# nubot-nudt/LCR-Net

Hardware: AMD Instinct MI355X
Metric: scans/s (120k-pt KITTI-shape scan -> 256-D descriptor) (higher is better)
Workload: dtype f32 (K-deep GEMMs, K >= 288 and N >= 64: fp32 operands as bf16 x 3 split, 6 of 9 products on the bf16 matrix cores, fp32 accumulate — error vs fp64 <= the fp32-MFMA kernel's; every other GEMM, KPConv and attention: fp32 MFMA); 1 GPU; configs[1]: batch of 8 synthetic 64-beam scans (~120k pts, 0.3 m voxel -> ~16k pts), voxelise + 3 subsamples + 10 radius searches + KPConv encoder + NetVLAD, seeded random weights; distinct_input_batches=4, streams=pre-processing stream (own host thread, 2 batches ahead) + 2 encoder stream(s), parallelism=scan-parallel x1, all-gather of descriptors

## Files before the change

lcr-net_amd/csrc/gemm_f32.hip:

```cpp
#include <cstdio>
#include <cstdlib>
#include <map>
#include <mutex>
#include <type_traits>

#include "common.h"

namespace lcr {

typedef float floatx16 __attribute__((ext_vector_type(16)));

constexpr int GM_BK = 32;
constexpr int GM_T = 256;

constexpr int GM_MAX_BATCH = 64;
struct GemmBatch {
  int     count;
  int     strided;
  int     k[GM_MAX_BATCH];
  int64_t a_off[GM_MAX_BATCH], b_off[GM_MAX_BATCH], c_off[GM_MAX_BATCH];
};

struct GemmEpilogue {
  const float*   bias;
// ... 728 lines not shown
      pin();
      mfma(a1[q], b1[q]);
      pin();
    }
#pragma unroll
    for (int q = 0; q < 4; ++q) {
      if (more && load) {
#pragma unroll
        for (int j = q; j < LPW; j += 4) issue_one(ST, j);
      }
      pin();
      mfma(a2[q], b2[q]);
      pin();
    }
    if (more && load) advance();
    mfma4(fa[3], fb[3]);
    if (more) {
#pragma unroll
      for (int q = 0; q < 4; ++q) fa[q] = na[q], fb[q] = nb[q];
    }
  };
  using I0 = std::integral_constant<int, 0>;
  using I1 = std::integral_constant<int, 1>;
  using I2 = std::integral_constant<int, 2>;
  int t = 0;
  for (; t + 6 <= nk; t += 3) {
    step(I0{}, std::true_type{}, t);
    step(I1{}, std::true_type{}, t + 1);
    step(I2{}, std::true_type{}, t + 2);
  }
  for (; t < nk; t += 3) {
    step(I0{}, std::false_type{}, t);
    if (t + 1 < nk) step(I1{}, std::false_type{}, t + 1);
    if (t + 2 < nk) step(I2{}, std::false_type{}, t + 2);
  }

  floatx16 accs[1] = {acc};
  gemm_epilogue<BM, BN, WM, WN, 1>(accs, C, M, N, m0, n0, m_tile, ep, bias_v, blk_first, blk_seg_start, blk_seg_end, wm, wn, lane);
}

template <int BM, int BN, int WM, int WN>
static int launch_gemm_deep(const float* A, const float* B, float* C, int64_t M, int N, int K, const GemmEpilogue& ep, hipStream_t st,
                            const uint16_t* amask = nullptr, int kshift = 0) {
  const int mt8 = (div_up(M, BM) + 7) / 8 * 8;
  if (amask)
    LCR_LAUNCH_TIMED((k_gemm_f32_deep<BM, BN, WM, WN, true>), dim3(mt8 * div_up(N, BN)), dim3(GM_T), 0, st, A, B, C, M, N, K, ep, amask, kshift);
  else
    LCR_LAUNCH_TIMED((k_gemm_f32_deep<BM, BN, WM, WN>), dim3(mt8 * div_up(N, BN)), dim3(GM_T), 0, st, A, B, C, M, N, K, ep, amask, kshift);
  return check_launch("lcr_gemm_f32");
}

typedef __bf16 bf16x8_t __attribute__((ext_vector_type(8)));
typedef __bf16 bf16x2_t __attribute__((ext_vector_type(2)));
typedef float f32x2_t __attribute__((ext_vector_type(2)));
typedef float f32x4_t __attribute__((ext_vector_type(4)));
typedef uint32_t u32x4_t __attribute__((ext_vector_type(4)));

__device__ __forceinline__ uint32_t pk_bf16(float a, float b) {
  f32x2_t v = {a, b};
  return __builtin_bit_cast(uint32_t, __builtin_convertvector(v, bf16x2_t));
}
__device__ __forceinline__ void split2(float x0, float x1, uint32_t& h1, uint32_t& h2, uint32_t& h3) {
  h1 = pk_bf16(x0, x1);
  const float r0 = fsub(x0, __uint_as_float(h1 << 16)), r1 = fsub(x1, __uint_as_float(h1 & 0xffff0000u));
  h2 = pk_bf16(r0, r1);
  const float s0 = fsub(r0, __uint_as_float(h2 << 16)), s1 = fsub(r1, __uint_as_float(h2 & 0xffff0000u));
  h3 = pk_bf16(s0, s1);
}

__global__ __launch_bounds__(256) void k_split_bf16x3(const float* __restrict__ w, int64_t n, uint16_t* __restrict__ planes) {
  for (int64_t i = (blockIdx.x * static_cast<int64_t>(blockDim.x) + threadIdx.x) * 2; i < n; i += static_cast<int64_t>(gridDim.x) * blockDim.x * 2) {
    const float x0 = w[i], x1 = i + 1 < n ? w[i + 1] : 0.f;
    uint32_t h1, h2, h3;
    split2(x0, x1, h1, h2, h3);
    planes[i] = static_cast<uint16_t>(h1), planes[n + i] = static_cast<uint16_t>(h2), planes[2 * n + i] = static_cast<uint16_t>(h3);
    if (i + 1 < n) planes[i + 1] = static_cast<uint16_t>(h1 >> 16), planes[n + i + 1] = static_cast<uint16_t>(h2 >> 16), planes[2 * n + i + 1] = static_cast<uint16_t>(h3 >> 16);
  }
}

__global__ __launch_bounds__(256) void k_split_bf16x3_tiles(const float* __restrict__ w, int N, int K, uint16_t* __restrict__ tiles) {
  const int KS = K / GM_BK;
  const int64_t blk = blockIdx.x;
  const int ct = static_cast<int>(blk / KS), ks = static_cast<int>(blk % KS);
  const int row = threadIdx.x >> 2, kc = threadIdx.x & 3;
  const int n = ct * 64 + row;
  u32x4_t p1 = {0u, 0u, 0u, 0u}, p2 = p1, p3 = p1;
  if (n < N) {
    const float* src = w + static_cast<int64_t>(n) * K + ks * GM_BK + kc * 8;
    const float4 x0 = ld4(src), x1 = ld4(src + 4);
    uint32_t h1, h2, h3;
    split2(x0.x, x0.y, h1, h2, h3), p1.x = h1, p2.x = h2, p3.x = h3;
    split2(x0.z, x0.w, h1, h2, h3), p1.y = h1, p2.y = h2, p3.y = h3;
    split2(x1.x, x1.y, h1, h2, h3), p1.z = h1, p2.z = h2, p3.z = h3;
    split2(x1.z, x1.w, h1, h2, h3), p1.w = h1, p2.w = h2, p3.w = h3;
  }
  char* dst = reinterpret_cast<char*>(tiles) + blk * 12288 + row * 64 + ((kc ^ ((row >> 2) & 3)) << 4);
  *reinterpret_cast<u32x4_t*>(dst) = p1;
  *reinterpret_cast<u32x4_t*>(dst + 4096) = p2;
  *reinterpret_cast<u32x4_t*>(dst + 8192) = p3;
}

template <int ABL, int NWM, int D = 2, bool MASK = false>
__global__ __launch_bounds__(128 * NWM, 2) void k_gemm_f32_bsplit_p(const float* __restrict__ A, const uint16_t* __restrict__ Bs, float* __restrict__ C,
                                                             int64_t M, int N, int K, GemmEpilogue ep, const uint16_t* __restrict__ amask,
                                                             int kshift) {
  constexpr int BM = 32 * NWM, BN = 64, RS = 64, T = 128 * NWM, PLA = BM * RS, STGA = 3 * PLA, PL = 64 * RS;
  constexpr int NPB = (768 + T - 1) / T;
  constexpr int STG = 3 * PL + (NPB * T - 768) * 16;
  __shared__ __attribute__((aligned(16))) char sA[2 * STGA];
  __shared__ __attribute__((aligned(16))) char sB[2 * STG];
  const int lane = threadIdx.x & 63, w = __builtin_amdgcn_readfirstlane(threadIdx.x >> 6);
  const int wm = w >> 1, wn = w & 1;
  const int ntn = (N + BN - 1) / BN;
  const int xcd = blockIdx.x & 7, slot = blockIdx.x >> 3;
  const int64_t m_tile = static_cast<int64_t>(slot / ntn) * 8 + xcd;
  const int64_t m0 = m_tile * BM;
  const int n0 = (slot % ntn) * BN;
  if (m0 >= M) return;
  const int srow = threadIdx.x >> 3, spc = threadIdx.x & 7;
  const float* ap[2];
  int soff[2];
  uint32_t aoff[2], rmask[2];
#pragma unroll
  for (int j = 0; j < 2; ++j) {
    const int r = srow + j * (T / 8);
    int64_t ga = m0 + r;
    ga = ga < M ? ga : M - 1;
    ap[j] = A + ga * K + spc * 4;
    if constexpr (MASK) {
      aoff[j] = static_cast<uint32_t>((ga * K + spc * 4) * 4);
      rmask[j] = amask[ga];
    } else {
      aoff[j] = rmask[j] = 0;
    }
    soff[j] = r * RS + (((spc >> 1) ^ ((r >> 2) & 3)) << 4) + (spc & 1) * 8;
  }
  const char* bp = reinterpret_cast<const char*>(Bs) + static_cast<int64_t>(n0 / 64) * (K / GM_BK) * 12288;
  int bsrc[NPB], bdst[NPB];
#pragma unroll
  for (int j = 0; j < NPB; ++j) {
    const int q = threadIdx.x + T * j;
    bsrc[j] = (q < 768 ? q : threadIdx.x) * 16;
    bdst[j] = q * 16;
  }
  const int fsw = ((lane & 31) >> 2) & 3, fc0 = ((lane >> 5) ^ fsw) << 4, fc1 = (((lane >> 5) + 2) ^ fsw) << 4;
  const int fa = (wm * 32 + (lane & 31)) * RS, fb = (wn * 32 + (lane & 31)) * RS;
  floatx16 acc, acc2;
#pragma unroll
  for (int r = 0; r < 16; ++r) acc[r] = 0.f, acc2[r] = 0.f;
  const int nk = K / GM_BK;
  f32x4_t ra[D][2];
  u32x4_t rb[D][NPB];
  __amdgpu_buffer_rsrc_t arsrc;
  if constexpr (MASK) arsrc = __builtin_amdgcn_make_buffer_rsrc(const_cast<float*>(A), 0, static_cast<int>(M * K * 4), 0x00020000);
  auto fetch = [&](auto st_c, int t) {
    constexpr int st = decltype(st_c)::value;
    const int tt = t < nk ? t : nk - 1;
    if constexpr (MASK) {
      const int kb = tt >> kshift;
#pragma unroll
      for (int j = 0; j < 2; ++j) {
        const uint32_t o = ((rmask[j] >> kb) & 1u) ? aoff[j] + static_cast<uint32_t>(tt * GM_BK * 4) : 0x80000000u;
        ra[st][j] = __builtin_bit_cast(f32x4_t, __builtin_amdgcn_raw_buffer_load_b128(arsrc, static_cast<int>(o), 0, 0));
      }
    } else {
      ra[st][0] = *reinterpret_cast<const f32x4_t*>(ap[0] + tt * GM_BK), ra[st][1] = *reinterpret_cast<const f32x4_t*>(ap[1] + tt * GM_BK);
    }
#pragma unroll
    for (int j = 0; j < NPB; ++j) rb[st][j] = *reinterpret_cast<const u32x4_t*>(bp + static_cast<int64_t>(tt) * 12288 + bsrc[j]);
  };
  auto park = [&](auto st_c, int lds_stage) {
    constexpr int st = decltype(st_c)::value;
    char* da = sA + lds_stage * STGA;
    char* db = sB + lds_stage * STG;
#pragma unroll
    for (int j = 0; j < 2; ++j) {
      uint32_t h1, h2, h3, g1, g2, g3;
      if constexpr (ABL & 2) {
        h1 = __float_as_uint(ra[st][j].x), h2 = __float_as_uint(ra[st][j].y), h3 = h1, g1 = __float_as_uint(ra[st][j].z), g2 = __float_as_uint(ra[st][j].w), g3 = g1;
      } else {
        split2(ra[st][j].x, ra[st][j].y, h1, h2, h3);
        split2(ra[st][j].z, ra[st][j].w, g1, g2, g3);
      }
      if constexpr (ABL & 4) {
        asm volatile("" ::"v"(h1), "v"(h2), "v"(h3), "v"(g1), "v"(g2), "v"(g3));
      } else {
        *reinterpret_cast<uint2*>(da + soff[j]) = make_uint2(h1, g1);
        *reinterpret_cast<uint2*>(da + PLA + soff[j]) = make_uint2(h2, g2);
        *reinterpret_cast<uint2*>(da + 2 * PLA + soff[j]) = make_uint2(h3, g3);
      }
    }
#pragma unroll
    for (int j = 0; j < NPB; ++j) {
      const u32x4_t v = rb[st][j];
      if constexpr (ABL & 4) {
        asm volatile("" ::"v"(v));
      } else {
        *reinterpret_cast<u32x4_t*>(db + bdst[j]) = v;
      }
    }
  };
  using I0 = std::integral_constant<int, 0>;
  fetch(I0{}, 0);
  if constexpr (D > 1) fetch(std::integral_constant<int, 1 % D>{}, 1);
  if constexpr (D > 2) fetch(std::integral_constant<int, 2 % D>{}, 2);
  if constexpr (D > 3) fetch(std::integral_constant<int, 3 % D>{}, 3);
  float bias_v[1];
  {
    const int col = n0 + wn * 32 + (lane & 31);
    bias_v[0] = (ep.bias && col < N) ? ep.bias[col] : 0.f;
  }
  int blk_first = 0;
  int64_t blk_seg_start = 0, blk_seg_end = 0;
  if (ep.stats != nullptr) {
    blk_seg_end = ep.seg_len[0];
    while (blk_first + 1 < ep.S && m0 >= blk_seg_end) {
      ++blk_first;
      blk_seg_start = blk_seg_end;
      blk_seg_end += ep.seg_len[blk_first];
    }
  }
  park(I0{}, 0);
  fetch(I0{}, D);
  __syncthreads();
  auto step = [&](auto lds_c, auto reg_c, int t) {
    constexpr int P = decltype(lds_c)::value;
    using NX = std::integral_constant<int, (decltype(reg_c)::value + 1) % D>;
    const char* la = sA + P * STGA + fa;
    const char* lb = sB + P * STG + fb;
    bf16x8_t a0[3], b0[3], a1[3], b1[3];
    auto mm = [&](const bf16x8_t& x, const bf16x8_t& y, floatx16& c) {
      if constexpr (ABL & 1) {
        asm volatile("" ::"v"(x), "v"(y));
      } else {
        c = __builtin_amdgcn_mfma_f32_32x32x16_bf16(x, y, c, 0, 0, 0);
      }
    };
    if constexpr (ABL & 16) {
      u32x4_t z = {static_cast<uint32_t>(t), 0u, 0u, 0u};
      asm volatile("" : "+v"(z));
#pragma unroll
      for (int p = 0; p < 3; ++p) a0[p] = b0[p] = a1[p] = b1[p] = __builtin_bit_cast(bf16x8_t, z);
      (void)la, (void)lb;
    } else {
#pragma unroll
      for (int p = 0; p < 3; ++p) {
        a0[p] = __builtin_bit_cast(bf16x8_t, *reinterpret_cast<const u32x4_t*>(la + p * PLA + fc0));
        b0[p] = __builtin_bit_cast(bf16x8_t, *reinterpret_cast<const u32x4_t*>(lb + p * PL + fc0));
      }
#pragma unroll
      for (int p = 0; p < 3; ++p) {
        a1[p] = __builtin_bit_cast(bf16x8_t, *reinterpret_cast<const u32x4_t*>(la + p * PLA + fc1));
        b1[p] = __builtin_bit_cast(bf16x8_t, *reinterpret_cast<const u32x4_t*>(lb + p * PL + fc1));
      }
    }
    mm(a0[2], b0[0], acc);
    mm(a0[0], b0[2], acc2);
    mm(a0[1], b0[1], acc);
    mm(a0[1], b0[0], acc2);
    mm(a0[0], b0[1], acc);
    mm(a0[0], b0[0], acc2);
    park(NX{}, P ^ 1);
    mm(a1[2], b1[0], acc);
    mm(a1[0], b1[2], acc2);
    mm(a1[1], b1[1], acc);
    mm(a1[1], b1[0], acc2);
    mm(a1[0], b1[1], acc);
    mm(a1[0], b1[0], acc2);
    if constexpr (!(ABL & 8)) fetch(NX{}, t + 1 + D);
    __syncthreads();
  };
  static_assert(D == 2 || D == 4, "register stages");
  using I1 = std::integral_constant<int, 1>;
  using I2 = std::integral_constant<int, 2>;
  using I3 = std::integral_constant<int, 3>;
  int t = 0;
  if constexpr (D == 2) {
    for (; t + 2 <= nk; t += 2) {
      step(I0{}, I0{}, t);
      step(I1{}, I1{}, t + 1);
    }
    if (t < nk) step(I0{}, I0{}, t);
  } else {
    for (; t + 4 <= nk; t += 4) {
      step(I0{}, I0{}, t);
      step(I1{}, I1{}, t + 1);
      step(I0{}, I2{}, t + 2);
      step(I1{}, I3{}, t + 3);
    }
    if (t < nk) step(I0{}, I0{}, t);
    if (t + 1 < nk) step(I1{}, I1{}, t + 1);
    if (t + 2 < nk) step(I0{}, I2{}, t + 2);
  }
#pragma unroll
  for (int r = 0; r < 16; ++r) acc[r] += acc2[r];
  floatx16 accs[1] = {acc};
  gemm_epilogue<BM, BN, NWM, 2, 1>(accs, C, M, N, m0, n0, m_tile, ep, bias_v, blk_first, blk_seg_start, blk_seg_end, wm, wn, lane);
}

struct GemmStreamK {
  float*    partial;
  uint32_t* arrived;
  int       U;
};

template <int BM, int BN, int WM, int WN>
__global__ __launch_bounds__(GM_T, 3) void k_gemm_f32_sk(const float* __restrict__ A, const float* __restrict__ B, float* __restrict__ C,
                                                         int64_t M, int N, int K, GemmEpilogue ep, GemmStreamK sk) {
  static_assert(WM * WN == 4 && BM == 32 * WM, "one 32-row MFMA tile per wavefront along M");
  constexpr int LDA = BM + 1, LDB = BN + 4;
  constexpr int NT = BN / (32 * WN);
  __shared__ __attribute__((aligned(16))) float As[2][GM_BK * LDA];
  __shared__ __attribute__((aligned(16))) float Bs[2][GM_BK * LDB];
  const int lane = threadIdx.x & 63, w = __builtin_amdgcn_readfirstlane(threadIdx.x >> 6);
  const int wm = w / WN, wn = w % WN;
  const int ntn = (N + BN - 1) / BN;
  const int64_t mt = (M + BM - 1) / BM;
  const int xcd = blockIdx.x & 7, u = blockIdx.x >> 3;
  const int64_t mt_x = mt > xcd ? (mt - xcd + 7) / 8 : 0;
  const int nk = (K + GM_BK - 1) / GM_BK;
  const int64_t I = mt_x * ntn * nk;
  auto first_it = [&](int uu) { return static_cast<int64_t>(uu) * I / sk.U; };
  const int64_t it_begin = first_it(u), it_end = first_it(u + 1);
  LoaderT<BM, LDA, true> la[2];
  LoaderN<BN, LDB, true> lb[2];
  const int a_off = (lane >> 5) * LDA + wm * 32 + (lane & 31);
  const int b_off = (lane >> 5) * LDB + wn * (32 * NT) + (lane & 31);
  constexpr int PIECE = NT * 16 * GM_T;
  __shared__ unsigned s_arrived;

  int64_t it = it_begin;
  while (it < it_end) {
    const int64_t lt = it / nk;
    const int ks = static_cast<int>(it - lt * nk);
    const int ns = static_cast<int>(min(static_cast<int64_t>(nk - ks), it_end - it));
    const int64_t m_tile = (lt / ntn) * 8 + xcd;
    const int64_t m0 = m_tile * BM;
    const int n0 = static_cast<int>(lt % ntn) * BN;
    const int k_begin = ks * GM_BK;
    auto gload = [&](int k0, int r) {
      la[r].load(A, M, K, m0, k0);
      lb[r].load(B, N, K, n0, k0);
    };
    floatx16 acc[NT];
#pragma unroll
    for (int j = 0; j < NT; ++j)
#pragma unroll
      for (int r = 0; r < 16; ++r) acc[j][r] = 0.f;
    gload(k_begin, 0);
    gload(k_begin + GM_BK, 1);
    const bool covers_end = ks + ns == nk, covers_start = ks == 0;
    float bias_v[NT];
#pragma unroll
    for (int j = 0; j < NT; ++j) {
      const int col = n0 + wn * (32 * NT) + j * 32 + (lane & 31);
      bias_v[j] = (ep.bias && col < N) ? ep.bias[col] : 0.f;
    }
    int blk_first = 0;
    int64_t blk_seg_start = 0, blk_seg_end = 0;
    la[0].store(As[0]);
    lb[0].store(Bs[0]);
    __syncthreads();

    constexpr int KK = GM_BK / 2;
    constexpr int PF = NT == 1 ? KK : (NT == 2 ? 8 : 4);
    constexpr int PA = BM * 8 / GM_T, PB = BN * 8 / GM_T;
    constexpr int ST0 = KK - (PA + PB) - 1 > 2 ? (KK - (PA + PB)) / 2 : 1;
    auto step = [&](auto buf_c, auto full_c, int t) {
      constexpr int BUF = decltype(buf_c)::value;
      constexpr bool FULL = decltype(full_c)::value;
      if (FULL || t + 2 < ns) gload(k_begin + (t + 2) * GM_BK, BUF);
      const bool do_store = FULL || t + 1 < ns;
      const float* as = As[BUF] + a_off;
      const float* bs = Bs[BUF] + b_off;
      float af[PF], bf[PF][NT];
#pragma unroll
      for (int d = 0; d < PF; ++d) {
        af[d] = as[d * 2 * LDA];
#pragma unroll
        for (int j = 0; j < NT; ++j) bf[d][j] = bs[d * 2 * LDB + j * 32];
// ... 235 lines not shown
    set_error("lcr_gemm_f32: bad argument");
    return LCR_EARG;
  }
  if (stats && (!seg_len || S < 1 || groups < 1 || N % groups != 0)) {
    set_error("lcr_gemm_f32: statistics need seg_len, S >= 1 and groups dividing N");
    return LCR_EARG;
  }
  if (stats) {
    const int gs = N / groups;
    if ((gs & (gs - 1)) != 0) {
      set_error("lcr_gemm_f32: channels per group must be a power of two");
      return LCR_EARG;
    }
  }
  hipStream_t st = static_cast<hipStream_t>(stream);
  KernelTimerScope timed(KT_GEMM, st, M, N, K);
  if (M == 0) return LCR_OK;
  GemmEpilogue ep{bias, rowdiv, seg_len, S, groups, stats};
  const int64_t lda = transA ? M : K, ldb = transB ? K : N;
  const bool vec = (lda % 4 == 0) && (ldb % 4 == 0) && (reinterpret_cast<uintptr_t>(A) % 16 == 0) && (reinterpret_cast<uintptr_t>(B) % 16 == 0);
  switch (gemm_form(M, N, K, transA, transB, vec)) {
    case GF_SCALAR: return launch_gemm<128, 64, 4, 1, false>(A, B, C, M, N, K, transA, transB, ep, st);
    case GF_FORCED_TILE:
      switch (g_force_tile) {
        case 1: return launch_gemm<128, 128, 4, 1, true>(A, B, C, M, N, K, transA, transB, ep, st);
        case 2: return launch_gemm<128, 64, 4, 1, true>(A, B, C, M, N, K, transA, transB, ep, st);
        case 3: return launch_gemm<128, 32, 4, 1, true>(A, B, C, M, N, K, transA, transB, ep, st);
        case 4: return launch_gemm<64, 64, 2, 2, true>(A, B, C, M, N, K, transA, transB, ep, st);
        default: return launch_gemm<64, 128, 2, 2, true>(A, B, C, M, N, K, transA, transB, ep, st);
      }
    case GF_SHORT:
      if (N <= 32) return launch_gemm<128, 32, 4, 1, true, true>(A, B, C, M, N, K, transA, transB, ep, st);
      return launch_gemm<64, 64, 2, 2, true, true>(A, B, C, M, N, K, transA, transB, ep, st);
    case GF_DEEP:
      if (N <= 32) return launch_gemm_deep<128, 32, 4, 1>(A, B, C, M, N, K, ep, st);
      return launch_gemm_deep<64, 64, 2, 2>(A, B, C, M, N, K, ep, st);
    case GF_STREAMK: return launch_gemm_sk(A, B, C, M, N, K, ep, st);
    case GF_TILE: break;
  }
  if (N <= 32) return launch_gemm<128, 32, 4, 1, true>(A, B, C, M, N, K, transA, transB, ep, st);
  const int64_t b128 = (M + 127) / 128, nb128 = (N + 127) / 128;
  if (K >= 512 && b128 * nb128 >= 512) return launch_gemm<128, 128, 4, 1, true>(A, B, C, M, N, K, transA, transB, ep, st);
  return launch_gemm<64, 64, 2, 2, true>(A, B, C, M, N, K, transA, transB, ep, st);
}

extern "C" int lcr_split_bf16x3(const float* w, int64_t n, uint16_t* planes, void* stream) {
  if (!w || !planes || n < 0) {
    set_error("lcr_split_bf16x3: bad argument");
    return LCR_EARG;
  }
  if (n == 0) return LCR_OK;
  hipLaunchKernelGGL(k_split_bf16x3, dim3(min(div_up(n, 512), 2048)), dim3(256), 0, static_cast<hipStream_t>(stream), w, n, planes);
  return check_launch("lcr_split_bf16x3");
}

extern "C" int lcr_split_bf16x3_tiles(const float* w, int N, int K, uint16_t* tiles, void* stream) {
  if (!w || !tiles || N < 1 || K < GM_BK || K % GM_BK != 0 || reinterpret_cast<uintptr_t>(w) % 16 != 0 || reinterpret_cast<uintptr_t>(tiles) % 16 != 0) {
    set_error("lcr_split_bf16x3_tiles: needs K %% 32 == 0 and 16-byte aligned buffers");
    return LCR_EARG;
  }
  hipLaunchKernelGGL(k_split_bf16x3_tiles, dim3(div_up(N, 64) * (K / GM_BK)), dim3(256), 0, static_cast<hipStream_t>(stream), w, N, K, tiles);
  return check_launch("lcr_split_bf16x3_tiles");
}

static int bsplit_impl(const float* A, const uint16_t* Bs, float* C, int64_t M, int N, int K, const float* bias, const float* rowdiv,
                       const int64_t* seg_len, int S, int groups, double* stats, const uint16_t* amask, int kshift, void* stream) {
  if (!A || !Bs || !C || M < 0 || N <= 0 || K <= 0 || K % GM_BK != 0 || reinterpret_cast<uintptr_t>(A) % 16 != 0 || reinterpret_cast<uintptr_t>(Bs) % 16 != 0 ||
      K < GM_BK) {
    set_error("lcr_gemm_f32_bsplit: needs K %% 32 == 0 and 16-byte aligned operands");
    return LCR_EARG;
  }
  if (stats && (!seg_len || S < 1 || groups < 1 || N % groups != 0 || ((N / groups) & (N / groups - 1)) != 0)) {
    set_error("lcr_gemm_f32_bsplit: statistics need seg_len, S >= 1 and groups dividing N into power-of-two sized groups");
    return LCR_EARG;
  }
  hipStream_t st = static_cast<hipStream_t>(stream);
  KernelTimerScope timed(KT_GEMM, st, M, N, K);
  if (M == 0) return LCR_OK;
  GemmEpilogue ep{bias, rowdiv, seg_len, S, groups, stats};
  const int mt8 = (div_up(M, 64) + 7) / 8 * 8;
  static const int abl = getenv("LCR_SPLIT_ABL") ? atoi(getenv("LCR_SPLIT_ABL")) : 0;
  const dim3 grid(mt8 * div_up(N, 64)), block(256);
  if (amask) {
    LCR_LAUNCH_TIMED((k_gemm_f32_bsplit_p<0, 2, 2, true>), grid, block, 0, st, A, Bs, C, M, N, K, ep, amask, kshift);
    return check_launch("lcr_gemm_f32_bsplit_masked");
  }
  switch (abl) {
    case 1: LCR_LAUNCH_TIMED((k_gemm_f32_bsplit_p<1, 2>), grid, block, 0, st, A, Bs, C, M, N, K, ep, amask, kshift); break;
    case 2: LCR_LAUNCH_TIMED((k_gemm_f32_bsplit_p<2, 2>), grid, block, 0, st, A, Bs, C, M, N, K, ep, amask, kshift); break;
    case 4: LCR_LAUNCH_TIMED((k_gemm_f32_bsplit_p<4, 2>), grid, block, 0, st, A, Bs, C, M, N, K, ep, amask, kshift); break;
    case 8: LCR_LAUNCH_TIMED((k_gemm_f32_bsplit_p<8, 2>), grid, block, 0, st, A, Bs, C, M, N, K, ep, amask, kshift); break;
    case 16: LCR_LAUNCH_TIMED((k_gemm_f32_bsplit_p<16, 2>), grid, block, 0, st, A, Bs, C, M, N, K, ep, amask, kshift); break;
    case 23: LCR_LAUNCH_TIMED((k_gemm_f32_bsplit_p<23, 2>), grid, block, 0, st, A, Bs, C, M, N, K, ep, amask, kshift); break;
    case 30: LCR_LAUNCH_TIMED((k_gemm_f32_bsplit_p<30, 2>), grid, block, 0, st, A, Bs, C, M, N, K, ep, amask, kshift); break;
    default: LCR_LAUNCH_TIMED((k_gemm_f32_bsplit_p<0, 2>), grid, block, 0, st, A, Bs, C, M, N, K, ep, amask, kshift); break;
  }
  return check_launch("lcr_gemm_f32_bsplit");
}

extern "C" int lcr_gemm_f32_bsplit(const float* A, const uint16_t* Bs, float* C, int64_t M, int N, int K, const float* bias, const float* rowdiv,
                                   const int64_t* seg_len, int S, int groups, double* stats, void* stream) {
  return bsplit_impl(A, Bs, C, M, N, K, bias, rowdiv, seg_len, S, groups, stats, nullptr, 0, stream);
}

static int mask_kshift(int K, int block_k) {
  for (int s = 0; s <= 3; ++s)
    if (block_k == (GM_BK << s)) return K <= 16 * block_k ? s : -1;
  return -1;
}

extern "C" int lcr_gemm_f32_bsplit_masked(const float* A, const uint16_t* Bs, float* C, int64_t M, int N, int K, const float* bias,
                                          const float* rowdiv, const int64_t* seg_len, int S, int groups, double* stats, const uint16_t* row_mask,
                                          int block_k, void* stream) {
  const int ks = mask_kshift(K, block_k);
  if (!row_mask || ks < 0 || M * static_cast<int64_t>(K) >= (int64_t(1) << 29)) {
    set_error("lcr_gemm_f32_bsplit_masked: needs a row mask, block_k = 32 << s (s <= 3) with K <= 16 block_k, and M*K < 2^29");
    return LCR_EARG;
  }
  return bsplit_impl(A, Bs, C, M, N, K, bias, rowdiv, seg_len, S, groups, stats, row_mask, ks, stream);
}

extern "C" int lcr_kpconv_mask_ok(int64_t M, int N, int K, int split) {
  static const bool off = getenv("LCR_KP_MASK") && atoi(getenv("LCR_KP_MASK")) == 0;
  if (off || M <= 0 || N <= 0 || K % 15 != 0 || mask_kshift(K, K / 15) < 0) return 0;
  if (split) return M * static_cast<int64_t>(K) < (int64_t(1) << 29);
  return gemm_form(M, N, K, 0, 1, true) == GF_DEEP;
}

extern "C" int lcr_gemm_f32_masked(const float* A, const float* B, float* C, int64_t M, int N, int K, const float* bias, const float* rowdiv,
                                   const int64_t* seg_len, int S, int groups, double* stats, const uint16_t* row_mask, int block_k, void* stream) {
  const int ks = mask_kshift(K, block_k);
  if (!A || !B || !C || !row_mask || M < 0 || N <= 0 || K <= 0 || K % GM_BK != 0 || ks < 0 || M * static_cast<int64_t>(K) >= (int64_t(1) << 30) ||
      static_cast<int64_t>(N) * K >= (int64_t(1) << 30) || reinterpret_cast<uintptr_t>(A) % 16 != 0 || reinterpret_cast<uintptr_t>(B) % 16 != 0) {
    set_error("lcr_gemm_f32_masked: needs a row mask, block_k = 32 << s (s <= 3) with K <= 16 block_k, K %% 32 == 0, M*K and N*K < 2^30, "
              "16-byte aligned operands");
    return LCR_EARG;
  }
  if (stats && (!seg_len || S < 1 || groups < 1 || N % groups != 0 || ((N / groups) & (N / groups - 1)) != 0)) {
    set_error("lcr_gemm_f32_masked: statistics need seg_len, S >= 1 and groups dividing N into power-of-two sized groups");
    return LCR_EARG;
  }
  hipStream_t st = static_cast<hipStream_t>(stream);
  KernelTimerScope timed(KT_GEMM, st, M, N, K);
  if (M == 0) return LCR_OK;
  GemmEpilogue ep{bias, rowdiv, seg_len, S, groups, stats};
  if (N <= 32) return launch_gemm_deep<128, 32, 4, 1>(A, B, C, M, N, K, ep, st, row_mask, ks);
  return launch_gemm_deep<64, 64, 2, 2>(A, B, C, M, N, K, ep, st, row_mask, ks);
}

extern "C" int lcr_gemm_f32_batched_ta(const float* A, const float* B, float* C, int64_t M, int N, int count, const int* k_host,
                                       const int64_t* a_off_host, const int64_t* b_off_host, const int64_t* c_off_host, void* stream) {
  if (!A || !B || !C || M <= 0 || N <= 0 || count < 1 || count > GM_MAX_BATCH || !k_host || !a_off_host || !b_off_host || !c_off_host) {
    set_error("lcr_gemm_f32_batched_ta: bad argument (count <= %d)", GM_MAX_BATCH);
    return LCR_EARG;
  }
  GemmBatch bt = {};
  bt.count = count;
  for (int i = 0; i < count; ++i) {
    bt.k[i] = k_host[i];
    bt.a_off[i] = a_off_host[i];
    bt.b_off[i] = b_off_host[i];
    bt.c_off[i] = c_off_host[i];
    if (a_off_host[i] % 4 || b_off_host[i] % 4 || k_host[i] < 1) {
      set_error("lcr_gemm_f32_batched_ta: offsets must be multiples of 4 floats and K >= 1");
      return LCR_EARG;
    }
  }
  if ((M % 4) || (N % 4)) {
    set_error("lcr_gemm_f32_batched_ta: M and N must be multiples of 4");
    return LCR_EARG;
  }
  GemmEpilogue ep{nullptr, nullptr, nullptr, 0, 0, nullptr};
  return launch_gemm<64, 64, 2, 2, true>(A, B, C, M, N,  1, 1, 0, ep, static_cast<hipStream_t>(stream), &bt);
}

extern "C" int lcr_gemm_f32_strided_batched(const float* A, const float* B, float* C, int64_t M, int N, int K, int transA, int transB,
                                            int64_t strideA, int64_t strideB, int64_t strideC, int count, void* stream) {
  if (!A || !B || !C || M <= 0 || N <= 0 || K <= 0 || count < 1 || count > 65535 || (strideA % 4) || (strideB % 4)) {
// ... 23 lines not shown
```

lcr-net_amd/functional.py:

```python
import ctypes
import os
import threading

import numpy as np
import torch

from . import _lib

GN_EPS = 1e-5
GN_REPLICAS = 8


class KernelTimer:
    KINDS = {"gemm": 0, "kpconv_aggregate": 1, "radius_query": 2, "attention": 3, "kpconv_fused": 4, "sinkhorn": 5}

    def __init__(self, names):
        self.names = set(names)
        self._cache = None

    def summary(self):
        return {k: [(b, m) for b, _, m in v] for k, v in self.records().items()}

    def records(self):
        if self._cache is None:
# ... 116 lines not shown
    return K // 15


def _gemm_masked(a, b, trans_b, trans_a, bias, rowdiv, seg_len, groups, row_mask):
    _lib.require_cuda(a, b)
    assert trans_b and not trans_a, "the masked form takes A [M,K] and B [N,K]"
    assert a.dtype == torch.float32 and b.dtype == torch.float32 and a.is_contiguous() and b.is_contiguous()
    block_k = _mask_args(a, row_mask)
    M, K = a.shape
    N = b.shape[0]
    assert b.shape[1] == K, "inner dimensions differ"
    c = torch.empty((M, N), dtype=torch.float32, device=a.device)
    stats, S = None, 0
    if groups:
        seg_len = _seg(seg_len, M, a.device)
        S = seg_len.numel()
        stats = _zero_stats(S, groups, a.device)
    _timed("gemm", lambda: _lib.check(_lib.lib().lcr_gemm_f32_masked(
        _lib.ptr(a), _lib.ptr(b), _lib.ptr(c), M, N, K, _lib.ptr(bias), _lib.ptr(rowdiv), _lib.ptr(seg_len) if groups else None, S,
        int(groups), _lib.ptr(stats), _lib.ptr(row_mask), block_k, _lib.stream_ptr(a.device)), "lcr_gemm_f32_masked"), meta=(M, N, K))
    return c, stats


_GEMM_SPLIT = [os.environ.get("LCR_GEMM_SPLIT", "1") not in ("", "0")]


def gemm_split_enabled():
    return _GEMM_SPLIT[0]


def set_gemm_split(on):
    _GEMM_SPLIT[0] = bool(on)


def gemm_split_ok(N, K):
    return K >= 288 and K % 32 == 0 and N >= 64


derived_lock = threading.RLock()


class WeightStamp:
    __slots__ = ("ref", "ptr", "ver", "dev")

    def __init__(self, t):
        import weakref
        self.ref, self.ptr, self.ver, self.dev = weakref.ref(t), t.data_ptr(), t._version, t.device

    def same(self, t):
        return self.ref is not None and self.ref() is t and self.ptr == t.data_ptr() and self.ver == t._version and self.dev == t.device

    def __reduce__(self):
        return (_dead_stamp, ())


def _dead_stamp():
    s = WeightStamp.__new__(WeightStamp)
    s.ref, s.ptr, s.ver, s.dev = None, 0, -1, None
    return s


def drop_derived(module, *names):
    for n in names:
        if n in module.__dict__:
            module.__dict__[n] = None



def publish_derived(t):
    torch.cuda.current_stream(t.device).synchronize()
    return t


def split_bf16x3(w):
    w = w.detach().contiguous()
    N, K = w.shape
    assert K % 32 == 0
    tiles = torch.empty(((N + 63) // 64, K // 32, 3, 64, 32), dtype=torch.int16, device=w.device)
    _lib.check(_lib.lib().lcr_split_bf16x3_tiles(_lib.ptr(w), int(N), int(K), _lib.ptr(tiles), _lib.stream_ptr(w.device)), "lcr_split_bf16x3_tiles")
    tiles.lcr_n = int(N)
    return tiles


def unsplit_bf16x3(tiles):
    CT, KS = tiles.shape[0], tiles.shape[1]
    t = tiles.view(CT, KS, 3, 64, 4, 8)
    row = torch.arange(64, device=tiles.device)
    phys = torch.arange(4, device=tiles.device)[None, :] ^ ((row >> 2) & 3)[:, None]
    t = torch.gather(t, 4, phys.view(1, 1, 1, 64, 4, 1).expand(CT, KS, 3, 64, 4, 8))
    t = t.reshape(CT, KS, 3, 64, 32).permute(2, 0, 3, 1, 4).reshape(3, CT * 64, KS * 32)
    return t[:, :tiles.lcr_n].contiguous().view(torch.bfloat16).float()


def gemm_bsplit(a, planes, bias=None, rowdiv=None, seg_len=None, groups=0, row_mask=None):
    _lib.require_cuda(a, planes)
    assert a.dtype == torch.float32 and a.is_contiguous() and planes.dtype == torch.int16 and planes.is_contiguous() and planes.dim() == 5
    M, K = a.shape
    N = planes.lcr_n
    assert planes.shape[1] * 32 == K and planes.shape[0] == (N + 63) // 64, "inner dimensions differ"
    c = torch.empty((M, N), dtype=torch.float32, device=a.device)
    stats, S = None, 0
    if groups:
        seg_len = _seg(seg_len, M, a.device)
        S = seg_len.numel()
        stats = _zero_stats(S, groups, a.device)
    if row_mask is not None:
        block_k = _mask_args(a, row_mask)
        _lib.check(_lib.lib().lcr_gemm_f32_bsplit_masked(_lib.ptr(a), _lib.ptr(planes), _lib.ptr(c), M, N, K, _lib.ptr(bias), _lib.ptr(rowdiv),
                                                         _lib.ptr(seg_len) if groups else None, S, int(groups), _lib.ptr(stats),
                                                         _lib.ptr(row_mask), block_k, _lib.stream_ptr(a.device)), "lcr_gemm_f32_bsplit_masked")
        return c, stats
    _lib.check(_lib.lib().lcr_gemm_f32_bsplit(_lib.ptr(a), _lib.ptr(planes), _lib.ptr(c), M, N, K, _lib.ptr(bias), _lib.ptr(rowdiv),
                                              _lib.ptr(seg_len) if groups else None, S, int(groups), _lib.ptr(stats), _lib.stream_ptr(a.device)),
               "lcr_gemm_f32_bsplit")
    return c, stats


ANORM_MAX_K, ANORM_MIN_SEG_ROWS = 256, 64


def gemm_anorm_ok(K, N):
    return K <= ANORM_MAX_K and K % 4 == 0 and N > 32


def gemm_anorm(a, a_stats, a_gamma, a_beta, a_groups, weight, bias=None, seg_len=None, groups=0, slope=0.1):
    _lib.require_cuda(a, weight)
    assert a.dtype == torch.float32 and weight.dtype == torch.float32 and a.is_contiguous() and weight.is_contiguous()
    M, K = a.shape
    N = weight.shape[0]
    assert weight.shape[1] == K and gemm_anorm_ok(K, N)
    c = torch.empty((M, N), dtype=torch.float32, device=a.device)
    seg_len = _seg(seg_len, M, a.device)
    S = seg_len.numel()
    stats = _zero_stats(S, groups, a.device) if groups else None
    _timed("gemm", lambda: _lib.check(_lib.lib().lcr_gemm_f32_anorm(
        _lib.ptr(a), _lib.ptr(weight), _lib.ptr(c), M, N, K, _lib.ptr(bias), _lib.ptr(a_stats), _lib.ptr(a_gamma), _lib.ptr(a_beta),
        int(a_groups), GN_EPS, float(slope), _lib.ptr(seg_len), S, int(groups), _lib.ptr(stats), _lib.stream_ptr(a.device)),
        "lcr_gemm_f32_anorm"), meta=(M, N, K))
    return c, stats


def groupnorm_stats(x, groups, seg_len=None):
    seg_len = _seg(seg_len, x.shape[0], x.device)
    stats = _zero_stats(seg_len.numel(), groups, x.device)
    _lib.check(_lib.lib().lcr_groupnorm_stats(_lib.ptr(x), x.shape[0], x.shape[1], groups, _lib.ptr(seg_len), seg_len.numel(),
                                              _lib.ptr(stats), _lib.stream_ptr(x.device)), "lcr_groupnorm_stats")
    return stats


def groupnorm_apply(x, stats, gamma, beta, groups, seg_len=None, res=None, res_norm=None, slope=0.1, act=True, want_pos=False):
    seg_len = _seg(seg_len, x.shape[0], x.device)
    y = torch.empty_like(x)
    pos = torch.empty((x.shape[0],), dtype=torch.uint8, device=x.device) if want_pos else None
    rs, rg, rb = res_norm if res_norm is not None else (None, None, None)
    _lib.check(_lib.lib().lcr_groupnorm_apply(_lib.ptr(x), _lib.ptr(stats), _lib.ptr(gamma), _lib.ptr(beta), _lib.ptr(res), _lib.ptr(rs),
                                              _lib.ptr(rg), _lib.ptr(rb), _lib.ptr(y), x.shape[0], x.shape[1], groups, _lib.ptr(seg_len),
                                              seg_len.numel(), GN_EPS, float(slope), int(act), _lib.ptr(pos),
                                              _lib.stream_ptr(x.device)), "lcr_groupnorm_apply")
    return (y, pos) if want_pos else y


def row_positive(x):
    pos = torch.empty((x.shape[0],), dtype=torch.uint8, device=x.device)
    _lib.check(_lib.lib().lcr_row_positive(_lib.ptr(x), x.shape[0], x.shape[1], _lib.ptr(pos), _lib.stream_ptr(x.device)), "lcr_row_positive")
    return pos


def _kp_host(kernel_points):
    kp = np.ascontiguousarray(kernel_points, dtype=np.float32)
    assert kp.shape == (15, 3)
    return kp


def kpconv_aggregate(s_feats, s_pos, q_points, s_points, idx, kernel_points_host, sigma, order=None, emit_mask=False):
# ... 915 lines not shown
```

Baseline: 2982 scans/s.

## Feed pre-split B fragments directly from global into 16x16 MFMA registers, bypassing LDS

Reorders the pre-split bf16x3 weight tiles so each wave can load its B fragments straight from global memory into registers in MFMA 16x16x32 operand order, which removes the B staging through LDS. The kernel now uses one 64x64 tile per 256-thread block, with each wave owning a 16-column slice, and switches from 32x32x16 to 16x16x32 bf16 MFMAs. The result is reshuffled through LDS so the existing epilogue can be reused. This cuts LDS traffic and size so three blocks can fit per CU, at the cost of an extra LDS round trip in the epilogue, more A-fragment LDS reads per wave, and a layout change that must stay consistent with the unsplit helper.

```diff
diff --git a/lcr-net_amd/csrc/gemm_f32.hip b/lcr-net_amd/csrc/gemm_f32.hip
--- a/lcr-net_amd/csrc/gemm_f32.hip
+++ b/lcr-net_amd/csrc/gemm_f32.hip
@@ -834,7 +834,8 @@
   const int KS = K / GM_BK;
   const int64_t blk = blockIdx.x;
   const int ct = static_cast<int>(blk / KS), ks = static_cast<int>(blk % KS);
-  const int row = threadIdx.x >> 2, kc = threadIdx.x & 3;
+  const int fl = threadIdx.x & 63, wn = threadIdx.x >> 6;
+  const int row = wn * 16 + (fl & 15), kc = fl >> 4;
   const int n = ct * 64 + row;
   u32x4_t p1 = {0u, 0u, 0u, 0u}, p2 = p1, p3 = p1;
   if (n < N) {
@@ -846,23 +847,19 @@
     split2(x1.x, x1.y, h1, h2, h3), p1.z = h1, p2.z = h2, p3.z = h3;
     split2(x1.z, x1.w, h1, h2, h3), p1.w = h1, p2.w = h2, p3.w = h3;
   }
-  char* dst = reinterpret_cast<char*>(tiles) + blk * 12288 + row * 64 + ((kc ^ ((row >> 2) & 3)) << 4);
+  char* dst = reinterpret_cast<char*>(tiles) + blk * 12288 + wn * 3072 + fl * 16;
   *reinterpret_cast<u32x4_t*>(dst) = p1;
-  *reinterpret_cast<u32x4_t*>(dst + 4096) = p2;
-  *reinterpret_cast<u32x4_t*>(dst + 8192) = p3;
-}
-
-template <int ABL, int NWM, int D = 2, bool MASK = false>
-__global__ __launch_bounds__(128 * NWM, 2) void k_gemm_f32_bsplit_p(const float* __restrict__ A, const uint16_t* __restrict__ Bs, float* __restrict__ C,
-                                                             int64_t M, int N, int K, GemmEpilogue ep, const uint16_t* __restrict__ amask,
-                                                             int kshift) {
-  constexpr int BM = 32 * NWM, BN = 64, RS = 64, T = 128 * NWM, PLA = BM * RS, STGA = 3 * PLA, PL = 64 * RS;
-  constexpr int NPB = (768 + T - 1) / T;
-  constexpr int STG = 3 * PL + (NPB * T - 768) * 16;
+  *reinterpret_cast<u32x4_t*>(dst + 1024) = p2;
+  *reinterpret_cast<u32x4_t*>(dst + 2048) = p3;
+}
+
+template <int ABL, bool MASK = false>
+__global__ __launch_bounds__(256, 3) void k_gemm_f32_bsplit_p(const float* __restrict__ A, const uint16_t* __restrict__ Bs, float* __restrict__ C,
+                                                           int64_t M, int N, int K, GemmEpilogue ep, const uint16_t* __restrict__ amask,
+                                                           int kshift) {
+  constexpr int BM = 64, BN = 64, RS = 64, T = 256, PLA = BM * RS, STGA = 3 * PLA, D = 2;
   __shared__ __attribute__((aligned(16))) char sA[2 * STGA];
-  __shared__ __attribute__((aligned(16))) char sB[2 * STG];
-  const int lane = threadIdx.x & 63, w = __builtin_amdgcn_readfirstlane(threadIdx.x >> 6);
-  const int wm = w >> 1, wn = w & 1;
+  const int lane = threadIdx.x & 63, wn = __builtin_amdgcn_readfirstlane(threadIdx.x >> 6);
   const int ntn = (N + BN - 1) / BN;
   const int xcd = blockIdx.x & 7, slot = blockIdx.x >> 3;
   const int64_t m_tile = static_cast<int64_t>(slot / ntn) * 8 + xcd;
@@ -887,25 +884,17 @@
     }
     soff[j] = r * RS + (((spc >> 1) ^ ((r >> 2) & 3)) << 4) + (spc & 1) * 8;
   }
-  const char* bp = reinterpret_cast<const char*>(Bs) + static_cast<int64_t>(n0 / 64) * (K / GM_BK) * 12288;
-  int bsrc[NPB], bdst[NPB];
-#pragma unroll
-  for (int j = 0; j < NPB; ++j) {
-    const int q = threadIdx.x + T * j;
-    bsrc[j] = (q < 768 ? q : threadIdx.x) * 16;
-    bdst[j] = q * 16;
-  }
-  const int fsw = ((lane & 31) >> 2) & 3, fc0 = ((lane >> 5) ^ fsw) << 4, fc1 = (((lane >> 5) + 2) ^ fsw) << 4;
-  const int fa = (wm * 32 + (lane & 31)) * RS, fb = (wn * 32 + (lane & 31)) * RS;
-  floatx16 acc, acc2;
-#pragma unroll
-  for (int r = 0; r < 16; ++r) acc[r] = 0.f, acc2[r] = 0.f;
+  const char* bp = reinterpret_cast<const char*>(Bs) + static_cast<int64_t>(n0 / 64) * (K / GM_BK) * 12288 + wn * 3072 + lane * 16;
+  const int fa = (lane & 15) * RS + (((lane >> 4) ^ (((lane & 15) >> 2) & 3)) << 4);
+  f32x4_t acc[4], acc2[4];
+#pragma unroll
+  for (int b = 0; b < 4; ++b) acc[b] = acc2[b] = f32x4_t{0.f, 0.f, 0.f, 0.f};
   const int nk = K / GM_BK;
   f32x4_t ra[D][2];
-  u32x4_t rb[D][NPB];
+  u32x4_t rb[2][3];
   __amdgpu_buffer_rsrc_t arsrc;
   if constexpr (MASK) arsrc = __builtin_amdgcn_make_buffer_rsrc(const_cast<float*>(A), 0, static_cast<int>(M * K * 4), 0x00020000);
-  auto fetch = [&](auto st_c, int t) {
+  auto fetch_a = [&](auto st_c, int t) {
     constexpr int st = decltype(st_c)::value;
     const int tt = t < nk ? t : nk - 1;
     if constexpr (MASK) {
@@ -918,13 +907,16 @@
     } else {
       ra[st][0] = *reinterpret_cast<const f32x4_t*>(ap[0] + tt * GM_BK), ra[st][1] = *reinterpret_cast<const f32x4_t*>(ap[1] + tt * GM_BK);
     }
-#pragma unroll
-    for (int j = 0; j < NPB; ++j) rb[st][j] = *reinterpret_cast<const u32x4_t*>(bp + static_cast<int64_t>(tt) * 12288 + bsrc[j]);
+  };
+  auto fetch_b = [&](auto st_c, int t) {
+    constexpr int st = decltype(st_c)::value;
+    const int tt = t < nk ? t : nk - 1;
+#pragma unroll
+    for (int p = 0; p < 3; ++p) rb[st][p] = *reinterpret_cast<const u32x4_t*>(bp + static_cast<int64_t>(tt) * 12288 + p * 1024);
   };
   auto park = [&](auto st_c, int lds_stage) {
     constexpr int st = decltype(st_c)::value;
     char* da = sA + lds_stage * STGA;
-    char* db = sB + lds_stage * STG;
 #pragma unroll
     for (int j = 0; j < 2; ++j) {
       uint32_t h1, h2, h3, g1, g2, g3;
@@ -942,26 +934,17 @@
         *reinterpret_cast<uint2*>(da + 2 * PLA + soff[j]) = make_uint2(h3, g3);
       }
     }
-#pragma unroll
-    for (int j = 0; j < NPB; ++j) {
-      const u32x4_t v = rb[st][j];
-      if constexpr (ABL & 4) {
-        asm volatile("" ::"v"(v));
-      } else {
-        *reinterpret_cast<u32x4_t*>(db + bdst[j]) = v;
-      }
-    }
   };
   using I0 = std::integral_constant<int, 0>;
-  fetch(I0{}, 0);
-  if constexpr (D > 1) fetch(std::integral_constant<int, 1 % D>{}, 1);
-  if constexpr (D > 2) fetch(std::integral_constant<int, 2 % D>{}, 2);
-  if constexpr (D > 3) fetch(std::integral_constant<int, 3 % D>{}, 3);
+  using I1 = std::integral_constant<int, 1>;
   float bias_v[1];
   {
-    const int col = n0 + wn * 32 + (lane & 31);
+    const int col = n0 + (wn & 1) * 32 + (lane & 31);
     bias_v[0] = (ep.bias && col < N) ? ep.bias[col] : 0.f;
   }
+  fetch_a(I0{}, 0);
+  fetch_a(I1{}, 1);
+  fetch_b(I0{}, 0);
   int blk_first = 0;
   int64_t blk_seg_start = 0, blk_seg_end = 0;
   if (ep.stats != nullptr) {
@@ -973,81 +956,69 @@
     }
   }
   park(I0{}, 0);
-  fetch(I0{}, D);
+  fetch_a(I0{}, 2);
+  fetch_b(I1{}, 1);
   __syncthreads();
-  auto step = [&](auto lds_c, auto reg_c, int t) {
+  auto step = [&](auto lds_c, int t) {
     constexpr int P = decltype(lds_c)::value;
-    using NX = std::integral_constant<int, (decltype(reg_c)::value + 1) % D>;
+    using NX = std::integral_constant<int, P ^ 1>;
     const char* la = sA + P * STGA + fa;
-    const char* lb = sB + P * STG + fb;
-    bf16x8_t a0[3], b0[3], a1[3], b1[3];
-    auto mm = [&](const bf16x8_t& x, const bf16x8_t& y, floatx16& c) {
+    bf16x8_t a[4][3];
+    auto mm = [&](const bf16x8_t& x, const u32x4_t& y, f32x4_t& c) {
       if constexpr (ABL & 1) {
         asm volatile("" ::"v"(x), "v"(y));
       } else {
-        c = __builtin_amdgcn_mfma_f32_32x32x16_bf16(x, y, c, 0, 0, 0);
+        c = __builtin_amdgcn_mfma_f32_16x16x32_bf16(x, __builtin_bit_cast(bf16x8_t, y), c, 0, 0, 0);
       }
     };
     if constexpr (ABL & 16) {
       u32x4_t z = {static_cast<uint32_t>(t), 0u, 0u, 0u};
       asm volatile("" : "+v"(z));
 #pragma unroll
-      for (int p = 0; p < 3; ++p) a0[p] = b0[p] = a1[p] = b1[p] = __builtin_bit_cast(bf16x8_t, z);
-      (void)la, (void)lb;
+      for (int b = 0; b < 4; ++b)
+#pragma unroll
+        for (int p = 0; p < 3; ++p) a[b][p] = __builtin_bit_cast(bf16x8_t, z);
+      (void)la;
     } else {
 #pragma unroll
-      for (int p = 0; p < 3; ++p) {
-        a0[p] = __builtin_bit_cast(bf16x8_t, *reinterpret_cast<const u32x4_t*>(la + p * PLA + fc0));
-        b0[p] = __builtin_bit_cast(bf16x8_t, *reinterpret_cast<const u32x4_t*>(lb + p * PL + fc0));
-      }
-#pragma unroll
-      for (int p = 0; p < 3; ++p) {
-        a1[p] = __builtin_bit_cast(bf16x8_t, *reinterpret_cast<const u32x4_t*>(la + p * PLA + fc1));
-        b1[p] = __builtin_bit_cast(bf16x8_t, *reinterpret_cast<const u32x4_t*>(lb + p * PL + fc1));
-      }
-    }
-    mm(a0[2], b0[0], acc);
-    mm(a0[0], b0[2], acc2);
-    mm(a0[1], b0[1], acc);
-    mm(a0[1], b0[0], acc2);
-    mm(a0[0], b0[1], acc);
-    mm(a0[0], b0[0], acc2);
+      for (int b = 0; b < 4; ++b)
+#pragma unroll
+        for (int p = 0; p < 3; ++p) a[b][p] = __builtin_bit_cast(bf16x8_t, *reinterpret_cast<const u32x4_t*>(la + p * PLA + b * (16 * RS)));
+    }
+    const u32x4_t &b0 = rb[P][0], &b1 = rb[P][1], &b2 = rb[P][2];
+    auto six = [&](int b) {
+      mm(a[b][2], b0, acc[b]);
+      mm(a[b][0], b2, acc2[b]);
+      mm(a[b][1], b1, acc[b]);
+      mm(a[b][1], b0, acc2[b]);
+      mm(a[b][0], b1, acc[b]);
+      mm(a[b][0], b0, acc2[b]);
+    };
+    six(0), six(1);
     park(NX{}, P ^ 1);
-    mm(a1[2], b1[0], acc);
-    mm(a1[0], b1[2], acc2);
-    mm(a1[1], b1[1], acc);
-    mm(a1[1], b1[0], acc2);
-    mm(a1[0], b1[1], acc);
-    mm(a1[0], b1[0], acc2);
-    if constexpr (!(ABL & 8)) fetch(NX{}, t + 1 + D);
+    six(2), six(3);
+    if constexpr (!(ABL & 8)) fetch_a(NX{}, t + 3);
+    if constexpr (!(ABL & (8 | 32))) fetch_b(lds_c, t + 2);
     __syncthreads();
   };
-  static_assert(D == 2 || D == 4, "register stages");
-  using I1 = std::integral_constant<int, 1>;
-  using I2 = std::integral_constant<int, 2>;
-  using I3 = std::integral_constant<int, 3>;
   int t = 0;
-  if constexpr (D == 2) {
-    for (; t + 2 <= nk; t += 2) {
-      step(I0{}, I0{}, t);
-      step(I1{}, I1{}, t + 1);
-    }
-    if (t < nk) step(I0{}, I0{}, t);
-  } else {
-    for (; t + 4 <= nk; t += 4) {
-      step(I0{}, I0{}, t);
-      step(I1{}, I1{}, t + 1);
-      step(I0{}, I2{}, t + 2);
-      step(I1{}, I3{}, t + 3);
-    }
-    if (t < nk) step(I0{}, I0{}, t);
-    if (t + 1 < nk) step(I1{}, I1{}, t + 1);
-    if (t + 2 < nk) step(I0{}, I2{}, t + 2);
-  }
-#pragma unroll
-  for (int r = 0; r < 16; ++r) acc[r] += acc2[r];
-  floatx16 accs[1] = {acc};
-  gemm_epilogue<BM, BN, NWM, 2, 1>(accs, C, M, N, m0, n0, m_tile, ep, bias_v, blk_first, blk_seg_start, blk_seg_end, wm, wn, lane);
+  for (; t + 2 <= nk; t += 2) {
+    step(I0{}, t);
+    step(I1{}, t + 1);
+  }
+  if (t < nk) step(I0{}, t);
+  float* sC = reinterpret_cast<float*>(sA);
+  static_assert(64 * 65 * 4 <= 2 * STGA, "the output tile fits the A stages");
+#pragma unroll
+  for (int b = 0; b < 4; ++b)
+#pragma unroll
+    for (int r = 0; r < 4; ++r) sC[(16 * b + 4 * (lane >> 4) + r) * 65 + 16 * wn + (lane & 15)] = acc[b][r] + acc2[b][r];
+  __syncthreads();
+  const int wm2 = wn >> 1, wn2 = wn & 1;
+  floatx16 accs[1];
+#pragma unroll
+  for (int r = 0; r < 16; ++r) accs[0][r] = sC[(32 * wm2 + (r & 3) + 8 * (r >> 2) + 4 * (lane >> 5)) * 65 + 32 * wn2 + (lane & 31)];
+  gemm_epilogue<BM, BN, 2, 2, 1>(accs, C, M, N, m0, n0, m_tile, ep, bias_v, blk_first, blk_seg_start, blk_seg_end, wm2, wn2, lane);
 }
 
 struct GemmStreamK {
@@ -1449,18 +1420,19 @@
   static const int abl = getenv("LCR_SPLIT_ABL") ? atoi(getenv("LCR_SPLIT_ABL")) : 0;
   const dim3 grid(mt8 * div_up(N, 64)), block(256);
   if (amask) {
-    LCR_LAUNCH_TIMED((k_gemm_f32_bsplit_p<0, 2, 2, true>), grid, block, 0, st, A, Bs, C, M, N, K, ep, amask, kshift);
+    LCR_LAUNCH_TIMED((k_gemm_f32_bsplit_p<0, true>), grid, block, 0, st, A, Bs, C, M, N, K, ep, amask, kshift);
     return check_launch("lcr_gemm_f32_bsplit_masked");
   }
   switch (abl) {
-    case 1: LCR_LAUNCH_TIMED((k_gemm_f32_bsplit_p<1, 2>), grid, block, 0, st, A, Bs, C, M, N, K, ep, amask, kshift); break;
-    case 2: LCR_LAUNCH_TIMED((k_gemm_f32_bsplit_p<2, 2>), grid, block, 0, st, A, Bs, C, M, N, K, ep, amask, kshift); break;
-    case 4: LCR_LAUNCH_TIMED((k_gemm_f32_bsplit_p<4, 2>), grid, block, 0, st, A, Bs, C, M, N, K, ep, amask, kshift); break;
-    case 8: LCR_LAUNCH_TIMED((k_gemm_f32_bsplit_p<8, 2>), grid, block, 0, st, A, Bs, C, M, N, K, ep, amask, kshift); break;
-    case 16: LCR_LAUNCH_TIMED((k_gemm_f32_bsplit_p<16, 2>), grid, block, 0, st, A, Bs, C, M, N, K, ep, amask, kshift); break;
-    case 23: LCR_LAUNCH_TIMED((k_gemm_f32_bsplit_p<23, 2>), grid, block, 0, st, A, Bs, C, M, N, K, ep, amask, kshift); break;
-    case 30: LCR_LAUNCH_TIMED((k_gemm_f32_bsplit_p<30, 2>), grid, block, 0, st, A, Bs, C, M, N, K, ep, amask, kshift); break;
-    default: LCR_LAUNCH_TIMED((k_gemm_f32_bsplit_p<0, 2>), grid, block, 0, st, A, Bs, C, M, N, K, ep, amask, kshift); break;
+    case 1: LCR_LAUNCH_TIMED((k_gemm_f32_bsplit_p<1>), grid, block, 0, st, A, Bs, C, M, N, K, ep, amask, kshift); break;
+    case 2: LCR_LAUNCH_TIMED((k_gemm_f32_bsplit_p<2>), grid, block, 0, st, A, Bs, C, M, N, K, ep, amask, kshift); break;
+    case 4: LCR_LAUNCH_TIMED((k_gemm_f32_bsplit_p<4>), grid, block, 0, st, A, Bs, C, M, N, K, ep, amask, kshift); break;
+    case 8: LCR_LAUNCH_TIMED((k_gemm_f32_bsplit_p<8>), grid, block, 0, st, A, Bs, C, M, N, K, ep, amask, kshift); break;
+    case 16: LCR_LAUNCH_TIMED((k_gemm_f32_bsplit_p<16>), grid, block, 0, st, A, Bs, C, M, N, K, ep, amask, kshift); break;
+    case 23: LCR_LAUNCH_TIMED((k_gemm_f32_bsplit_p<23>), grid, block, 0, st, A, Bs, C, M, N, K, ep, amask, kshift); break;
+    case 30: LCR_LAUNCH_TIMED((k_gemm_f32_bsplit_p<30>), grid, block, 0, st, A, Bs, C, M, N, K, ep, amask, kshift); break;
+    case 32: LCR_LAUNCH_TIMED((k_gemm_f32_bsplit_p<32>), grid, block, 0, st, A, Bs, C, M, N, K, ep, amask, kshift); break;
+    default: LCR_LAUNCH_TIMED((k_gemm_f32_bsplit_p<0>), grid, block, 0, st, A, Bs, C, M, N, K, ep, amask, kshift); break;
   }
   return check_launch("lcr_gemm_f32_bsplit");
 }
diff --git a/lcr-net_amd/functional.py b/lcr-net_amd/functional.py
--- a/lcr-net_amd/functional.py
+++ b/lcr-net_amd/functional.py
@@ -222,14 +222,13 @@
     return tiles
 
 
-def unsplit_bf16x3(tiles):
+def unsplit_bf16x3(tiles, padded=False):
     CT, KS = tiles.shape[0], tiles.shape[1]
-    t = tiles.view(CT, KS, 3, 64, 4, 8)
-    row = torch.arange(64, device=tiles.device)
-    phys = torch.arange(4, device=tiles.device)[None, :] ^ ((row >> 2) & 3)[:, None]
-    t = torch.gather(t, 4, phys.view(1, 1, 1, 64, 4, 1).expand(CT, KS, 3, 64, 4, 8))
-    t = t.reshape(CT, KS, 3, 64, 32).permute(2, 0, 3, 1, 4).reshape(3, CT * 64, KS * 32)
-    return t[:, :tiles.lcr_n].contiguous().view(torch.bfloat16).float()
+    t = tiles.view(CT, KS, 4, 3, 4, 16, 8)
+    t = t.permute(3, 0, 2, 5, 1, 4, 6).reshape(3, CT * 64, KS * 32)
+    if not padded:
+        t = t[:, :tiles.lcr_n]
+    return t.contiguous().view(torch.bfloat16).float()
 
 
 def gemm_bsplit(a, planes, bias=None, rowdiv=None, seg_len=None, groups=0, row_mask=None):
```

Measured after the change: 3039 scans/s (median of 6 runs). 1.9% higher.
